# SorF520/D2R

Measured on AMD Instinct MI355X. Metric: samples/sec fwd+bwd, higher is better.
Workload: dtype fp16; 1 GPU; BASELINE configs[1]: synthetic MVSA-Single-style batch, per-GPU batch 32, seq_len 128, 197 image tokens, DR_step 3, 6 cells per routing layer, 3 classes, 12+12 encoder layers, random-init weights, dropout 0; step = fwd+bwd+grad-allreduce+AdamW; global_batch=32, seq_len=128, parallelism=dp1

## Files before the change

d2r_amd/csrc/gemm.hip:

```cpp
#include <stdlib.h>

#include <algorithm>
#include <mutex>
#include <vector>

#include "gemm_args.h"
#include "ktimer.h"

template <typename T, int LAYOUT, int BM, int BN, int WAVES_M, int WAVES_N, int NBUF, bool GROUPED = false>
__global__ __launch_bounds__(256) void gemm_kernel(GemmArgs g, GemmGroup grp) {
  constexpr bool IS_BF16 = sizeof(T) == 2;
  constexpr int BK = IS_BF16 ? 64 : 16;
  constexpr int VEC = 16 / sizeof(T);
  constexpr int NT = 256;
  static_assert(WAVES_M * WAVES_N == 4, "4 waves per workgroup");
  constexpr int WM = BM / WAVES_M, WN = BN / WAVES_N;
  constexpr int TM = WM / 16, TN = WN / 16;
  static_assert(WM % 16 == 0 && WN % 16 == 0, "wave tile must be a multiple of 16");
  constexpr bool A_KCONT = (LAYOUT != D2R_GEMM_TN);
  constexpr bool B_KCONT = (LAYOUT == D2R_GEMM_NT);
  constexpr int LDK = BK + (IS_BF16 ? 8 : 1);
  constexpr int LDA_T = BM + (IS_BF16 ? 8 : 16);
  constexpr int LDB_T = BN + (IS_BF16 ? 8 : 16);
  constexpr int SZ_A = A_KCONT ? BM * LDK : BK * LDA_T;
// ... 292 lines not shown
        if (g.P) store_c(g.P, g.c_dtype, ci, v);
        v = act_apply_cold(g.act, v);
        if (g.R) v += load_c(g.R, g.c_dtype, rz + (int64_t)row * g.ldr + col);
        if (g.beta != 0.f) v += g.beta * load_c(g.C, g.c_dtype, ci);
        store_c(g.C, g.c_dtype, ci, v);
      }
    }
  }
}

__global__ __launch_bounds__(256) void splitk_reduce_kernel(GemmArgs g) {
  const int64_t total = (int64_t)g.M * g.N;
  if (g.dbias) {
    const float* wb = g.ws + (int64_t)g.splits * total;
    for (int64_t m = (int64_t)blockIdx.x * 256 + threadIdx.x; m < g.M; m += (int64_t)gridDim.x * 256) {
      float s = 0.f;
      for (int k = 0; k < g.splits; ++k) s += wb[(int64_t)k * g.M + m];
      g.dbias[m] += s;
    }
  }
  for (int64_t idx = (int64_t)blockIdx.x * 256 + threadIdx.x; idx < total; idx += (int64_t)gridDim.x * 256) {
    float s = 0.f;
    for (int k0 = 0; k0 < g.splits; k0 += 8) {
      float t[8];
#pragma unroll
      for (int u = 0; u < 8; ++u) {
        const int k = k0 + u;
        t[u] = g.ws[(int64_t)(k < g.splits ? k : 0) * total + idx] * (k < g.splits ? 1.f : 0.f);
      }
#pragma unroll
      for (int u = 0; u < 8; ++u) s += t[u];
    }
    const int m = (int)(idx / g.N), n = (int)(idx - (int64_t)m * g.N);
    const int64_t ci = (int64_t)m * g.ldc + n;
    float v = g.alpha * s + (g.bias ? g.bias[n] : 0.f);
    if (g.P) store_c(g.P, g.c_dtype, ci, v);
    v = act_apply_cold(g.act, v);
    if (g.G) v *= act_grad_cold(g.gact, load_c(g.G, g.c_dtype, ci));
    if (g.R) v += load_c(g.R, g.c_dtype, (int64_t)m * g.ldr + n);
    if (g.beta != 0.f) v += g.beta * load_c(g.C, g.c_dtype, ci);
    store_c(g.C, g.c_dtype, ci, v);
  }
}

static int g_nbuf = 1;
static int g_vepi = 1;
static int g_tile = -1;
static int g_xcd = 1;
static int g_wgrad_glds = 1;
static int g_dbg = 0;
static int g_gemm8 = 1;
static int g_group = 1;
static int g_gemm8_wgrad = 1;
static int g_splitk = 1;
static int g_gemm8_min = 150;

thread_local int d2r_gemm_variant_tl = 0;

struct GemmTimerRec {
  int family;
  double flops, bytes;
  hipEvent_t e0, e1;
};
static std::vector<GemmTimerRec> g_timer_recs;
static std::mutex g_timer_mu;
static volatile int g_timer_on = 0;

static thread_local int g_timer_depth = 0;
D2RTimerScope::D2RTimerScope(hipStream_t stream, int fam, double fl, double by) : family(fam), flops(fl), bytes(by), st(stream) {
  if (fam < 10000) d2r_gemm_variant_tl = 0;
  if (g_timer_depth++ > 0) return;
  if (!g_timer_on) return;
  if (hipEventCreate(&e0) != hipSuccess) return;
  if (hipEventCreate(&e1) != hipSuccess) { (void)hipEventDestroy(e0); return; }
  (void)hipEventRecord(e0, st);
  armed = true;
}
D2RTimerScope::~D2RTimerScope() {
  --g_timer_depth;
  if (!armed) return;
  GemmTimerRec rec;
  rec.family = family < 10000 ? family + 100 * d2r_gemm_variant_tl : family;
  rec.flops = flops, rec.bytes = bytes, rec.e0 = e0, rec.e1 = e1;
  (void)hipEventRecord(e1, st);
  std::lock_guard<std::mutex> lk(g_timer_mu);
  g_timer_recs.push_back(rec);
}
typedef D2RTimerScope GemmTimerScope;

extern "C" int d2r_gemm_timer(int on) {
  std::lock_guard<std::mutex> lk(g_timer_mu);
  if (on) {
    for (auto& r : g_timer_recs) (void)hipEventDestroy(r.e0), (void)hipEventDestroy(r.e1);
    g_timer_recs.clear();
  }
  g_timer_on = on ? 1 : 0;
  return D2R_OK;
}

extern "C" int d2r_gemm_timer_read(int* family, double* flops, double* bytes, float* ms, int capacity) {
  std::lock_guard<std::mutex> lk(g_timer_mu);
  int n = 0;
  for (auto& r : g_timer_recs) {
    float t = 0.f;
    if (hipEventSynchronize(r.e1) == hipSuccess && hipEventElapsedTime(&t, r.e0, r.e1) == hipSuccess && n < capacity && family) {
      family[n] = r.family, flops[n] = r.flops, bytes[n] = r.bytes, ms[n] = t;
      ++n;
    }
    (void)hipEventDestroy(r.e0), (void)hipEventDestroy(r.e1);
  }
  const int total = (int)g_timer_recs.size();
  g_timer_recs.clear();
  return family ? n : total;
}
extern "C" void d2r_gemm_tuning(int nbuf, int vepi, int tile) {
  g_nbuf = nbuf & 0xff;
  g_xcd = (nbuf >> 8) & 1 ? 0 : 1;
  g_vepi = vepi;
  if (tile == 100 || tile == 101) g_wgrad_glds = tile - 100;
  else if (tile == 102 || tile == 103) g_gemm8_wgrad = tile - 102;
  else if (tile >= 110 && tile <= 113) g_gemm8 = tile - 110;
  else if (tile == 130 || tile == 131) g_splitk = tile - 130;
  else if (tile == 120 || tile == 121) g_group = tile - 120;
  else if (tile >= 2000) g_dbg = tile - 2000;
  else if (tile >= 1000) g_gemm8_min = tile - 1000;
  else g_tile = tile;
}

template <typename T, int LAYOUT, int BM, int BN, int WM_, int WN_>
static void launch_tile(const GemmArgs& a, int gz, hipStream_t st) {
  dim3 grid(d2r_cdiv(a.N, BN), d2r_cdiv(a.M, BM), gz);
  static const GemmGroup no_group = {};
  if (g_nbuf == 2) hipLaunchKernelGGL((gemm_kernel<T, LAYOUT, BM, BN, WM_, WN_, 2>), grid, dim3(256), 0, st, a, no_group);
  else hipLaunchKernelGGL((gemm_kernel<T, LAYOUT, BM, BN, WM_, WN_, 1>), grid, dim3(256), 0, st, a, no_group);
}

int d2r_gemm_glds_try(const GemmArgs& a, int layout, int batch, int bn, hipStream_t st);
int d2r_gemm8_fwd_ok(const GemmArgs& a, int layout, int batch);
int d2r_gemm8_fwd_launch(const GemmArgs* probs, int n, int layout, hipStream_t st);
int d2r_gemm8_wgrad_ok(int dtype, int M, int N, int K, int64_t lda, int64_t ldb, int64_t ldc, const void* A, const void* B, const void* C);
int d2r_gemm8_wgrad_launch(int dtype, int count, const int* M, const int* N, const int* K, const int64_t* lda, const int64_t* ldb, const int64_t* ldc,
                           const void* const* A, const void* const* B, float* const* C, float* const* dbias, float beta, hipStream_t st);
int d2r_gemm_glds_splitk_plan(const GemmArgs& a, int layout, int batch, size_t ws_bytes, size_t* slab_bytes);
int d2r_gemm_glds_splitk_launch(const GemmArgs& a, int layout, hipStream_t st);
static bool gemm8_pays(const GemmArgs& a) {
  if (g_gemm8 == 2 && (a.act != 0 || a.G != nullptr)) return false;
  if (g_gemm8 == 3 && (a.act != 0 || a.G != nullptr || a.R != nullptr || a.P != nullptr)) return false;
  const int64_t t = (int64_t)d2r_cdiv(a.M, 256) * d2r_cdiv(a.N, 256);
  if (t < g_gemm8_min) return false;
  const int64_t rounds = (t + 255) / 256;
  return t * 100 >= rounds * 256 * 70;
}
static int g_glds = 1;

template <int LAYOUT>
__global__ __launch_bounds__(256) void gemm_skinny_f32_kernel(GemmArgs g) {
  constexpr int MAXS = 12;
  __shared__ float red[4][2][16][17];
  const int tid = threadIdx.x, lane = tid & 63, wave = tid >> 6;
  const int fr = lane & 15, fq = lane >> 4;
  const int z = blockIdx.z, zb = z / g.nh, zh = z - zb * g.nh;
  const float* A = reinterpret_cast<const float*>(g.A) + zb * g.sAb + zh * g.sAh;
  const float* B = reinterpret_cast<const float*>(g.B) + zb * g.sBb + zh * g.sBh;
  const int n0 = blockIdx.x * 16;
  const int col = min(n0 + fr, g.N - 1);
  const int r0 = min(fr, g.M - 1), r1 = min(16 + fr, g.M - 1);
  const bool two = g.M > 16;
  f32x4 acc0 = {0.f, 0.f, 0.f, 0.f}, acc1 = {0.f, 0.f, 0.f, 0.f};
  const int k16 = g.K / 16, per = (k16 + 3) / 4;
  const int kbeg = min(wave * per, k16), kend = min(kbeg + per, k16);
  for (int s0 = kbeg; s0 < kbeg + per; s0 += MAXS) {
    const int ns = max(0, min(MAXS, kend - s0));
    f32x4 a0[MAXS], a1[MAXS], b[MAXS];
#pragma unroll
    for (int s = 0; s < MAXS; ++s) {
      if (s < ns) {
        const int k = (s0 + s) * 16 + fq * 4;
        a0[s] = *reinterpret_cast<const f32x4*>(A + (int64_t)r0 * g.lda + k);
        if (two) a1[s] = *reinterpret_cast<const f32x4*>(A + (int64_t)r1 * g.lda + k);
        if constexpr (LAYOUT == D2R_GEMM_NT) {
          b[s] = *reinterpret_cast<const f32x4*>(B + (int64_t)col * g.ldb + k);
        } else {
#pragma unroll
          for (int j = 0; j < 4; ++j) b[s][j] = B[(int64_t)(k + j) * g.ldb + col];
        }
      }
    }
#pragma unroll
    for (int s = 0; s < MAXS; ++s) {
      if (s < ns) {
#pragma unroll
        for (int j = 0; j < 4; ++j) {
          acc0 = __builtin_amdgcn_mfma_f32_16x16x4f32(a0[s][j], b[s][j], acc0, 0, 0, 0);
          if (two) acc1 = __builtin_amdgcn_mfma_f32_16x16x4f32(a1[s][j], b[s][j], acc1, 0, 0, 0);
        }
// ... 512 lines not shown
  for (int first = 0; first < count; first += D2R_GEMM_GROUP_MAX) {
    const int n = count - first < D2R_GEMM_GROUP_MAX ? count - first : D2R_GEMM_GROUP_MAX;
    GemmGroup grp = {};
    for (int i = 0; i < n; ++i) {
      grp.A[i] = A[first + i], grp.B[i] = B[first + i], grp.C[i] = C[first + i];
      grp.dbias[i] = dbias ? dbias[first + i] : nullptr;
    }
    GemmArgs a = base;
    a.dbias = dbias ? reinterpret_cast<float*>(1) : nullptr;
    if (sizeof(T) == 2 && g_wgrad_glds) {
      GemmArgs b = a;
      b.xcd = g_xcd;
      if (d2r_gemm_glds_wgrad_try(b, grp, n, st)) {
        if (int rc = d2r_check_launch("d2r_gemm_tn_grouped(glds)")) return rc;
        continue;
      }
    }
    dim3 grid(d2r_cdiv(a.N, 64), d2r_cdiv(a.M, 64), n);
    if (a.K >= 1 && a.K <= 64 && (int64_t)a.M * a.N >= 4096) {
      d2r_gemm_variant_tl = 33;
      hipLaunchKernelGGL((gemm_rank_tn_kernel<T, true>), grid, dim3(256), 0, st, a, grp);
      if (int rc = d2r_check_launch("d2r_gemm_tn_grouped(rank-K)")) return rc;
      continue;
    }
    if (grid.x >= 24 && grid.x % 8 == 0) a.xcd = 0;
    d2r_gemm_variant_tl = 21;
    hipLaunchKernelGGL((gemm_kernel<T, D2R_GEMM_TN, 64, 64, 2, 2, 1, true>), grid, dim3(256), 0, st, a, grp);
    if (int rc = d2r_check_launch("d2r_gemm_tn_grouped")) return rc;
  }
  return D2R_OK;
}

static int tn_grouped_same(int dtype, int M, int N, int K, int64_t lda, int64_t ldb, int64_t ldc, const void* const* h_A, const void* const* h_B,
                           float* const* h_C, float* const* h_dbias, int count, float beta, void* stream, bool allow8) {
  D2R_REQUIRE(h_A && h_B && h_C && count >= 0, "d2r_gemm_tn_grouped: null pointer array");
  D2R_REQUIRE(dtype == D2R_F32 || d2r_is16(dtype), "d2r_gemm_tn_grouped: bad dtype %d", dtype);
  D2R_REQUIRE(M >= 1 && N >= 1 && K >= 0 && lda >= M && ldb >= N && ldc >= N, "d2r_gemm_tn_grouped: bad shape");
  if (count == 0) return D2R_OK;
  const int64_t es = (int64_t)d2r_esize(dtype);
  GemmArgs a = {};
  a.M = M, a.N = N, a.K = K, a.nh = 1, a.splits = 1, a.lda = lda, a.ldb = ldb, a.ldc = ldc;
  a.alpha = 1.f, a.beta = beta, a.act = D2R_ACT_NONE, a.c_dtype = D2R_F32, a.dtype = dtype, a.xcd = g_xcd, a.grouped = 1, a.dbg = 0, a.band = 0;
  a.vecA = (lda * es) % 16 == 0, a.vecB = (ldb * es) % 16 == 0, a.vecC = 0;
  for (int i = 0; i < count; ++i) {
    D2R_REQUIRE(h_A[i] && h_B[i] && h_C[i] && (!h_dbias || h_dbias[i]), "d2r_gemm_tn_grouped: null operand in problem %d", i);
    a.vecA &= d2r_aligned16(h_A[i]) ? 1 : 0;
    a.vecB &= d2r_aligned16(h_B[i]) ? 1 : 0;
    for (int j = 0; j < i; ++j) {
      D2R_REQUIRE(h_C[i] != h_C[j], "d2r_gemm_tn_grouped: problems %d and %d write the same C", j, i);
      D2R_REQUIRE(!h_dbias || h_dbias[i] != h_dbias[j], "d2r_gemm_tn_grouped: problems %d and %d write the same dbias", j, i);
    }
  }
  hipStream_t st = reinterpret_cast<hipStream_t>(stream);
  GemmTimerScope timed(st, dtype * 8 + D2R_GEMM_TN * 2 + 1, 2.0 * count * M * N * (double)K,
                       (double)count * (((double)K * M + (double)K * N) * es + 2.0 * M * N * 4.0));
  if (allow8 && g_gemm8_wgrad && d2r_is16(dtype) && (int64_t)count * d2r_cdiv(M, 256) * d2r_cdiv(N, 256) >= 96) {
    bool ok = true;
    for (int i = 0; i < count && ok; ++i) ok = d2r_gemm8_wgrad_ok(dtype, M, N, K, lda, ldb, ldc, h_A[i], h_B[i], h_C[i]) != 0;
    if (ok) {
      std::vector<int> Ms(count, M), Ns(count, N), Ks(count, K);
      std::vector<int64_t> la(count, lda), lb(count, ldb), lc(count, ldc);
      d2r_gemm_variant_tl = 28;
      return d2r_gemm8_wgrad_launch(dtype, count, Ms.data(), Ns.data(), Ks.data(), la.data(), lb.data(), lc.data(), h_A, h_B, h_C, h_dbias, beta, st);
    }
  }
  if (dtype == D2R_BF16) return launch_grouped_tn<bf16_t>(a, h_A, h_B, h_C, h_dbias, count, st);
  if (dtype == D2R_F16) return launch_grouped_tn<f16_t>(a, h_A, h_B, h_C, h_dbias, count, st);
  return launch_grouped_tn<float>(a, h_A, h_B, h_C, h_dbias, count, st);
}

extern "C" int d2r_gemm_tn_grouped(int dtype, int M, int N, int K, int64_t lda, int64_t ldb, int64_t ldc, const void* const* h_A,
                                   const void* const* h_B, float* const* h_C, float* const* h_dbias, int count, float beta, void* stream) {
  return tn_grouped_same(dtype, M, N, K, lda, ldb, ldc, h_A, h_B, h_C, h_dbias, count, beta, stream, true);
}


extern "C" int d2r_gemm_tn_grouped_v(int dtype, int count, const int* M, const int* N, const int* K, const int64_t* lda, const int64_t* ldb,
                                     const int64_t* ldc, const void* const* h_A, const void* const* h_B, float* const* h_C,
                                     float* const* h_dbias, float beta, void* stream) {
  D2R_REQUIRE(count >= 0 && (count == 0 || (M && N && K && lda && ldb && ldc && h_A && h_B && h_C)), "d2r_gemm_tn_grouped_v: null array");
  D2R_REQUIRE(dtype == D2R_F32 || d2r_is16(dtype), "d2r_gemm_tn_grouped_v: bad dtype %d", dtype);
  hipStream_t st = reinterpret_cast<hipStream_t>(stream);
  std::vector<int> wide, rest;
  for (int i = 0; i < count; ++i) {
    D2R_REQUIRE(h_A[i] && h_B[i] && h_C[i] && (!h_dbias || h_dbias[i]), "d2r_gemm_tn_grouped_v: null operand in problem %d", i);
    D2R_REQUIRE(M[i] >= 1 && N[i] >= 1 && K[i] >= 0 && lda[i] >= M[i] && ldb[i] >= N[i] && ldc[i] >= N[i], "d2r_gemm_tn_grouped_v: bad shape in problem %d", i);
    for (int j = 0; j < i; ++j) {
      D2R_REQUIRE(h_C[i] != h_C[j], "d2r_gemm_tn_grouped_v: problems %d and %d write the same C", j, i);
      D2R_REQUIRE(!h_dbias || h_dbias[i] != h_dbias[j], "d2r_gemm_tn_grouped_v: problems %d and %d write the same dbias", j, i);
    }
    const bool w = g_gemm8_wgrad && d2r_gemm8_wgrad_ok(dtype, M[i], N[i], K[i], lda[i], ldb[i], ldc[i], h_A[i], h_B[i], h_C[i]);
    (w ? wide : rest).push_back(i);
  }
  int64_t wtiles = 0;
  for (int i : wide) wtiles += (int64_t)d2r_cdiv(M[i], 256) * d2r_cdiv(N[i], 256);
  if (wtiles < 96) {
    rest.insert(rest.end(), wide.begin(), wide.end());
    wide.clear();
  }
  if (!wide.empty()) {
    const int n = (int)wide.size();
    std::vector<int> Ms(n), Ns(n), Ks(n);
    std::vector<int64_t> la(n), lb(n), lc(n);
    std::vector<const void*> As(n), Bs(n);
    std::vector<float*> Cs(n), Ds(n);
    double flops = 0, bytes = 0;
    for (int k = 0; k < n; ++k) {
      const int i = wide[k];
      Ms[k] = M[i], Ns[k] = N[i], Ks[k] = K[i], la[k] = lda[i], lb[k] = ldb[i], lc[k] = ldc[i], As[k] = h_A[i], Bs[k] = h_B[i], Cs[k] = h_C[i];
      Ds[k] = h_dbias ? h_dbias[i] : nullptr;
      flops += 2.0 * M[i] * N[i] * (double)K[i];
      bytes += ((double)K[i] * M[i] + (double)K[i] * N[i]) * 2.0 + (beta != 0.f ? 2.0 : 1.0) * M[i] * N[i] * 4.0;
    }
    GemmTimerScope timed(st, dtype * 8 + D2R_GEMM_TN * 2 + 1, flops, bytes);
    d2r_gemm_variant_tl = 28;
    if (int rc = d2r_gemm8_wgrad_launch(dtype, n, Ms.data(), Ns.data(), Ks.data(), la.data(), lb.data(), lc.data(), As.data(), Bs.data(), Cs.data(),
                                        h_dbias ? Ds.data() : nullptr, beta, st))
      return rc;
  }
  std::vector<char> done(count, 0);
  for (size_t a = 0; a < rest.size(); ++a) {
    const int i = rest[a];
    if (done[i]) continue;
    std::vector<const void*> As, Bs;
    std::vector<float*> Cs, Ds;
    for (size_t b = a; b < rest.size(); ++b) {
      const int j = rest[b];
      if (done[j] || M[j] != M[i] || N[j] != N[i] || K[j] != K[i] || lda[j] != lda[i] || ldb[j] != ldb[i] || ldc[j] != ldc[i]) continue;
      done[j] = 1;
      As.push_back(h_A[j]), Bs.push_back(h_B[j]), Cs.push_back(h_C[j]), Ds.push_back(h_dbias ? h_dbias[j] : nullptr);
    }
    if (int rc = tn_grouped_same(dtype, M[i], N[i], K[i], lda[i], ldb[i], ldc[i], As.data(), Bs.data(), Cs.data(), h_dbias ? Ds.data() : nullptr,
                                 (int)As.size(), beta, stream, false))
      return rc;
  }
  return D2R_OK;
}


int d2r_gemm_glds_batched_tn_try(const GemmArgs& a, const GemmGroup& grp, int ngroups, hipStream_t st);
int d2r_gemm_tn_batched16(int dtype, int M, int m_store, int N, int K, int64_t lda, int64_t sAb, int64_t ldb, int64_t sBb, int64_t ldc,
                          int64_t sCb, const void* const* A, const void* const* B, void* const* C, int ngroups, int nb, void* stream) {
  D2R_REQUIRE(d2r_is16(dtype) && A && B && C && ngroups >= 1 && ngroups <= D2R_GEMM_GROUP_MAX && nb >= 1, "d2r_gemm_tn_batched16: bad arguments");
  D2R_REQUIRE(m_store >= 1 && m_store <= M && N >= 1 && K >= 1 && lda >= M && ldb >= N && ldc >= N, "d2r_gemm_tn_batched16: bad shape");
  hipStream_t st = reinterpret_cast<hipStream_t>(stream);
  GemmArgs a = {};
  a.M = M, a.m_store = m_store, a.N = N, a.K = K, a.nh = 1, a.splits = 1, a.lda = lda, a.ldb = ldb, a.ldc = ldc, a.sAb = sAb, a.sBb = sBb, a.sCb = sCb;
  a.alpha = 1.f, a.beta = 0.f, a.act = D2R_ACT_NONE, a.c_dtype = dtype, a.dtype = dtype, a.xcd = g_xcd, a.grouped = 1, a.gbatch = nb;
  auto ok16 = [](const void* p, int64_t ld, int64_t sb) { return d2r_aligned16(p) && (ld * 2) % 16 == 0 && (sb * 2) % 16 == 0; };
  a.vecA = a.vecB = a.vecC = 1;
  GemmGroup grp = {};
  for (int i = 0; i < ngroups; ++i) {
    D2R_REQUIRE(A[i] && B[i] && C[i], "d2r_gemm_tn_batched16: null operand in group %d", i);
    a.vecA &= ok16(A[i], lda, sAb) ? 1 : 0, a.vecB &= ok16(B[i], ldb, sBb) ? 1 : 0, a.vecC &= ok16(C[i], ldc, sCb) ? 1 : 0;
    grp.A[i] = A[i], grp.B[i] = B[i], grp.C[i] = C[i];
  }
  {
    GemmTimerScope timed(st, dtype * 8 + D2R_GEMM_TN * 2 + 1, 2.0 * ngroups * nb * (double)m_store * N * K,
                         (double)ngroups * nb * (((double)K * m_store + (double)K * N) * 2.0 + (double)m_store * N * 2.0));
    if (g_glds && d2r_gemm_glds_batched_tn_try(a, grp, ngroups, st)) return d2r_check_launch("d2r_gemm_tn_batched16(glds)");
  }
  for (int i = 0; i < ngroups; ++i) {
    d2r_gemm_desc d = {};
    d.dtype = d.c_dtype = dtype, d.layout = D2R_GEMM_TN, d.act = D2R_ACT_NONE, d.M = m_store, d.N = N, d.K = K, d.nb = nb, d.nh = 1, d.alpha = 1.f;
    d.A = A[i], d.lda = lda, d.sAb = sAb, d.B = B[i], d.ldb = ldb, d.sBb = sBb, d.C = C[i], d.ldc = ldc, d.sCb = sCb;
    if (int rc = d2r_gemm(&d, stream)) return rc;
  }
  return D2R_OK;
}
```

d2r_amd/csrc/gemm8.hip:

```cpp
#include "gemm_args.h"

#ifndef D2R_G8_STAMPS
#define D2R_G8_STAMPS 0
#endif

__device__ __attribute__((aligned(256))) unsigned char d2r_g8_zero_page[256];

namespace {

constexpr int G8_UNIT = 16384;
constexpr int G8_A0 = 0, G8_B0 = G8_UNIT, G8_B1 = 2 * G8_UNIT, G8_A1 = 3 * G8_UNIT, G8_BUF = 4 * G8_UNIT;
constexpr int G8_SMEM = 2 * G8_BUF;

__device__ __forceinline__ int g8_kswz(int k) { return ((k & 3) | ((k >> 1) & 4)) << 1; }

template <int OFF, typename V8>
__device__ __forceinline__ V8 g8_read128(unsigned addr) {
  V8 r;
  asm volatile("ds_read_b128 %0, %1 offset:%2" : "=v"(r) : "v"(addr), "n"(OFF));
  return r;
}
template <int OFF, typename V4>
__device__ __forceinline__ V4 g8_read_tr(unsigned addr) {
  V4 r;
  asm volatile("ds_read_b64_tr_b16 %0, %1 offset:%2" : "=v"(r) : "v"(addr), "n"(OFF));
  return r;
}

__device__ __forceinline__ void g8_barrier() {
  asm volatile("s_barrier" ::: "memory");
  __builtin_amdgcn_sched_barrier(0);
}
__device__ __forceinline__ void g8_lgkm0() {
  asm volatile("s_waitcnt lgkmcnt(0)" ::: "memory");
  __builtin_amdgcn_sched_barrier(0);
}
__device__ __forceinline__ void g8_wait_units(int units) {
  if (units >= 4) asm volatile("s_waitcnt vmcnt(8)" ::: "memory");
  else if (units == 3) asm volatile("s_waitcnt vmcnt(6)" ::: "memory");
  else if (units == 2) asm volatile("s_waitcnt vmcnt(4)" ::: "memory");
  else if (units == 1) asm volatile("s_waitcnt vmcnt(2)" ::: "memory");
  else asm volatile("s_waitcnt vmcnt(0)" ::: "memory");
  __builtin_amdgcn_sched_barrier(0);
}

template <typename E, int LAYOUT, bool BIAS>
__device__ __forceinline__ void g8_main(const E* __restrict__ A, const E* __restrict__ B, int M, int N, int K, int64_t lda, int64_t ldb,
                                        int m0, int n0, unsigned char* smem, f32x4 (&acc)[8][4], f32x4 (&accb)[2], bool do_bias,
                                        unsigned long long* stamps) {
  typedef typename H16<E>::v8 h8;
  typedef typename H16<E>::v4 h4;
  constexpr bool A_KC = LAYOUT != D2R_GEMM_TN, B_KC = LAYOUT == D2R_GEMM_NT;
  constexpr bool RAGGED = LAYOUT == D2R_GEMM_TN;
// ... 172 lines not shown
    G8_MFMA(0, 0, bf0);
    G8_BIAS(0);
    G8_STAMP(sb + 1);
    g8_barrier();
    G8_STAMP(sb + 2);
    G8_READ_B(G8_B1, bf1);
    __builtin_amdgcn_sched_barrier(0);
    if (more1) issueA(1, buf ^ 1, t + 1);
    __builtin_amdgcn_sched_barrier(0);
    g8_wait_units(more1 ? INF : 0);
    g8_barrier();
    G8_STAMP(sb + 3);
    g8_lgkm0();
    G8_MFMA(0, 1, bf1);
    G8_STAMP(sb + 4);
    g8_barrier();
    G8_STAMP(sb + 5);
    G8_READ_A(G8_A1);
    __builtin_amdgcn_sched_barrier(0);
    if (more2) issueA(0, buf, t + 2);
    __builtin_amdgcn_sched_barrier(0);
    g8_barrier();
    G8_STAMP(sb + 6);
    g8_lgkm0();
    G8_MFMA(1, 1, bf1);
    G8_BIAS(1);
    G8_STAMP(sb + 7);
    g8_barrier();
    G8_STAMP(sb + 8);
    if (more2) issueB(0, buf, t + 2);
    __builtin_amdgcn_sched_barrier(0);
    if (more1) g8_wait_units(more2 ? INF : 2);
    g8_barrier();
    G8_STAMP(sb + 9);
    G8_MFMA(1, 0, bf0);
    G8_STAMP(sb + 10);
    g8_barrier();
    G8_STAMP(sb + 11);
  }
  if (wr == 0) g8_barrier();
  G8_STAMP(63);
  if (stamps && blockIdx.x == 0) {
    asm volatile("s_waitcnt vmcnt(0)" ::: "memory");
    stamps[wave * 64 + lane] = ((unsigned long long)st_hi << 32) | st_lo;
  }
#undef G8_STAMP
#undef G8_READ_A
#undef G8_READ_B
#undef G8_MFMA
#undef G8_BIAS
}

constexpr int G8_WMAX = 40;
struct G8ProbW {
  const void* A;
  const void* B;
  float* C;
  float* dbias;
  int M, N, K, lda, ldb, ldc, tn, pad;
};
struct G8GroupW {
  int nprob, ntiles;
  float beta;
  int xcd;
  unsigned long long* stamps;
  int tile_end[G8_WMAX];
  G8ProbW p[G8_WMAX];
};

__device__ __forceinline__ int g8_xcd_remap(int id, int nwg, int enable) {
  if (!enable || nwg < 16) return id;
  const int q = nwg >> 3, r = nwg & 7, xcd = id & 7, k = id >> 3;
  return (xcd < r ? xcd * (q + 1) : r * (q + 1) + (xcd - r) * q) + k;
}

template <typename E>
__global__ __launch_bounds__(512) void gemm8_wgrad_kernel(const G8GroupW g) {
  __shared__ __attribute__((aligned(1024))) unsigned char smem[G8_SMEM];
  const int L = g8_xcd_remap(blockIdx.x, g.ntiles, g.xcd);
  int lo = 0, hi = g.nprob - 1;
  while (lo < hi) {
    const int mid = (lo + hi) >> 1;
    if (L < g.tile_end[mid]) hi = mid;
    else lo = mid + 1;
  }
  const int z = __builtin_amdgcn_readfirstlane(lo);
  const G8ProbW& P = g.p[z];
  const int first = z ? g.tile_end[z - 1] : 0;
  const int rem = L - first, tile_m = rem / P.tn, tile_n = rem - tile_m * P.tn;
  const int m0 = tile_m * 256, n0 = tile_n * 256;
  const int M = P.M, N = P.N;
  f32x4 acc[8][4], accb[2];
#pragma unroll
  for (int i = 0; i < 8; ++i)
#pragma unroll
    for (int j = 0; j < 4; ++j) acc[i][j] = f32x4{0.f, 0.f, 0.f, 0.f};
  accb[0] = accb[1] = f32x4{0.f, 0.f, 0.f, 0.f};
  const bool do_bias = P.dbias != nullptr && tile_n == 0;
  g8_main<E, D2R_GEMM_TN, true>(reinterpret_cast<const E*>(P.A), reinterpret_cast<const E*>(P.B), M, N, P.K, P.lda, P.ldb, m0, n0, smem, acc, accb,
                                     do_bias, D2R_G8_STAMPS ? g.stamps : nullptr);

  const int lane = threadIdx.x & 63, wave = __builtin_amdgcn_readfirstlane(threadIdx.x >> 6), wr = wave >> 2, wc = wave & 3;
  const int fr = lane & 15, fq = lane >> 4;
  float* C = P.C;
  const int64_t ldc = P.ldc;
  const float beta = g.beta;
#pragma unroll
  for (int mh = 0; mh < 2; ++mh) {
    f32x4 old[4][4];
    if (beta != 0.f) {
#pragma unroll
      for (int i = 0; i < 4; ++i) {
        const int row = min(m0 + wr * 128 + mh * 64 + i * 16 + fr, M - 1);
#pragma unroll
        for (int nj = 0; nj < 4; ++nj) {
          const int col = min(n0 + wc * 64 + (nj >> 1) * 32 + (nj & 1) * 16 + fq * 4, N - 4);
          old[i][nj] = *reinterpret_cast<const f32x4*>(C + (int64_t)row * ldc + col);
        }
      }
    }
#pragma unroll
    for (int i = 0; i < 4; ++i) {
      const int row = m0 + wr * 128 + mh * 64 + i * 16 + fr;
#pragma unroll
      for (int nj = 0; nj < 4; ++nj) {
        const int col = n0 + wc * 64 + (nj >> 1) * 32 + (nj & 1) * 16 + fq * 4;
        f32x4 v = acc[mh * 4 + i][nj];
        if (beta != 0.f) v = f32x4{v[0] + beta * old[i][nj][0], v[1] + beta * old[i][nj][1], v[2] + beta * old[i][nj][2], v[3] + beta * old[i][nj][3]};
        if (row < M && col + 4 <= N) *reinterpret_cast<f32x4*>(C + (int64_t)row * ldc + col) = v;
      }
    }
  }
// ... 121 lines not shown
void launch_fwd(const G8GroupF& g, int layout, hipStream_t st) {
  if (layout == D2R_GEMM_NT) hipLaunchKernelGGL((gemm8_fwd_kernel<E, D2R_GEMM_NT>), dim3(g.ntiles), dim3(512), 0, st, g);
  else hipLaunchKernelGGL((gemm8_fwd_kernel<E, D2R_GEMM_NN>), dim3(g.ntiles), dim3(512), 0, st, g);
}

}

static unsigned long long* g8_stamps = nullptr;
extern "C" void d2r_gemm8_debug_stamps(unsigned long long* dst) { g8_stamps = dst; }
int d2r_gemm8_fwd_ok(const GemmArgs& a, int layout, int batch) {
  if (!d2r_is16(a.dtype) || a.c_dtype != a.dtype || batch != 1 || layout == D2R_GEMM_TN) return 0;
  if (a.K % 64 != 0 || a.K < 128 || a.M < 256 || a.N < 256 || a.N % 8 != 0) return 0;
  if (!a.vecA || !a.vecB || !a.vecC || a.dbias) return 0;
  return 1;
}

static void g8_fill_prob(G8ProbF& p, const GemmArgs& a) {
  p.A = a.A, p.B = a.B, p.C = a.C, p.bias = a.bias, p.R = a.R, p.P = a.P, p.G = a.G;
  p.M = a.M, p.N = a.N, p.K = a.K, p.lda = (int)a.lda, p.ldb = (int)a.ldb, p.ldc = (int)a.ldc, p.ldr = (int)a.ldr;
  p.tn = d2r_cdiv(a.N, 256);
  p.alpha = a.alpha, p.beta = a.beta, p.act = a.act, p.gact = a.gact, p.pad = 0;
  const int64_t panel = (int64_t)256 * a.K * 2;
  int band = (int)((int64_t)(1536 << 10) / (panel > 0 ? panel : 1));
  if (band < 2) band = 2;
  p.band = (p.tn > band && (int64_t)p.tn * panel > (3 << 20)) ? band : 0;
}

int d2r_gemm8_fwd_launch(const GemmArgs* probs, int n, int layout, hipStream_t st) {
  if (n < 1 || n > G8_FMAX) return d2r_fail(D2R_ERR_INVALID, "d2r_gemm8_fwd_launch: %d problems (1..%d)", n, G8_FMAX);
  G8GroupF g = {};
  g.nprob = n, g.xcd = 1;
  int tiles = 0;
  for (int i = 0; i < n; ++i) {
    g8_fill_prob(g.p[i], probs[i]);
    tiles += d2r_cdiv(probs[i].M, 256) * g.p[i].tn;
    g.tile_end[i] = tiles;
  }
  for (int i = n; i < G8_FMAX; ++i) g.tile_end[i] = tiles;
  g.ntiles = tiles;
  g.stamps = g8_stamps;
  if (probs[0].dtype == D2R_F16) launch_fwd<f16_t>(g, layout, st);
  else launch_fwd<bf16_t>(g, layout, st);
  return d2r_check_launch("d2r_gemm8(fwd)");
}

int d2r_gemm8_wgrad_ok(int dtype, int M, int N, int K, int64_t lda, int64_t ldb, int64_t ldc, const void* A, const void* B, const void* C) {
  if (!d2r_is16(dtype) || M < 128 || N < 128 || K < 128 || M % 8 != 0 || N % 8 != 0) return 0;
  if ((lda * 2) % 16 != 0 || (ldb * 2) % 16 != 0 || (ldc * 4) % 16 != 0) return 0;
  if (!d2r_aligned16(A) || !d2r_aligned16(B) || !d2r_aligned16(C)) return 0;
  if (lda >= ((int64_t)1 << 31) || ldb >= ((int64_t)1 << 31) || ldc >= ((int64_t)1 << 31)) return 0;
  return 1;
}

int d2r_gemm8_wgrad_launch(int dtype, int count, const int* M, const int* N, const int* K, const int64_t* lda, const int64_t* ldb, const int64_t* ldc,
                           const void* const* A, const void* const* B, float* const* C, float* const* dbias, float beta, hipStream_t st) {
  for (int first = 0; first < count; first += G8_WMAX) {
    const int n = count - first < G8_WMAX ? count - first : G8_WMAX;
    G8GroupW g = {};
    g.nprob = n, g.beta = beta, g.xcd = 1;
    int tiles = 0;
    for (int i = 0; i < n; ++i) {
      const int s = first + i;
      G8ProbW& p = g.p[i];
      p.A = A[s], p.B = B[s], p.C = C[s], p.dbias = dbias ? dbias[s] : nullptr;
      p.M = M[s], p.N = N[s], p.K = K[s], p.lda = (int)lda[s], p.ldb = (int)ldb[s], p.ldc = (int)ldc[s];
      p.tn = d2r_cdiv(N[s], 256), p.pad = 0;
      tiles += d2r_cdiv(M[s], 256) * p.tn;
      g.tile_end[i] = tiles;
    }
    for (int i = n; i < G8_WMAX; ++i) g.tile_end[i] = tiles;
    g.ntiles = tiles;
    g.stamps = g8_stamps;
    if (dtype == D2R_F16) hipLaunchKernelGGL((gemm8_wgrad_kernel<f16_t>), dim3(tiles), dim3(512), 0, st, g);
    else hipLaunchKernelGGL((gemm8_wgrad_kernel<bf16_t>), dim3(tiles), dim3(512), 0, st, g);
    if (int rc = d2r_check_launch("d2r_gemm8(wgrad)")) return rc;
  }
  return D2R_OK;
}

extern "C" int d2r_gemm8_probe_fwd(int dtype, int layout, int M, int N, int K, const void* A, int64_t lda, const void* B, int64_t ldb, void* C,
                                   int64_t ldc, const float* bias, int act, int nrep, void* stream) {
  GemmArgs a = {};
  a.A = A, a.B = B, a.C = C, a.bias = bias, a.M = M, a.N = N, a.K = K, a.lda = lda, a.ldb = ldb, a.ldc = ldc, a.ldr = ldc;
  a.alpha = 1.f, a.beta = 0.f, a.act = act, a.dtype = dtype, a.c_dtype = dtype, a.vecA = a.vecB = a.vecC = 1;
  if (!d2r_gemm8_fwd_ok(a, layout, 1)) return d2r_fail(D2R_ERR_INVALID, "d2r_gemm8_probe_fwd: shape not eligible");
  GemmArgs probs[G8_FMAX];
  if (nrep < 1 || nrep > G8_FMAX) return d2r_fail(D2R_ERR_INVALID, "d2r_gemm8_probe_fwd: nrep");
  for (int i = 0; i < nrep; ++i) probs[i] = a;
  return d2r_gemm8_fwd_launch(probs, nrep, layout, reinterpret_cast<hipStream_t>(stream));
}
```

d2r_amd/csrc/gemm_args.h:

```cpp
#pragma once
#include "common.h"

typedef __attribute__((ext_vector_type(8))) __bf16 bf16x8;
typedef __attribute__((ext_vector_type(4))) __bf16 bf16x4;
typedef __attribute__((ext_vector_type(8))) _Float16 f16x8;
typedef __attribute__((ext_vector_type(4))) _Float16 f16x4;
typedef __attribute__((ext_vector_type(4))) float f32x4;

template <typename T> struct H16;
template <> struct H16<bf16_t> {
  typedef bf16x8 v8;
  typedef bf16x4 v4;
  static constexpr int DT = D2R_BF16;
  static __device__ __forceinline__ f32x4 mfma32(v8 a, v8 b, f32x4 c) { return __builtin_amdgcn_mfma_f32_16x16x32_bf16(a, b, c, 0, 0, 0); }
  static __device__ __forceinline__ f32x4 mfma16(v4 a, v4 b, f32x4 c) { return __builtin_amdgcn_mfma_f32_16x16x16bf16_1k(a, b, c, 0, 0, 0); }
  static __device__ __forceinline__ v4 tr_read(const bf16_t* lds) {
    typedef __attribute__((address_space(3))) v4 lds_v4;
    return __builtin_amdgcn_ds_read_tr16_b64_v4bf16((lds_v4*)lds);
  }
};
template <> struct H16<f16_t> {
  typedef f16x8 v8;
  typedef f16x4 v4;
  static constexpr int DT = D2R_F16;
  static __device__ __forceinline__ f32x4 mfma32(v8 a, v8 b, f32x4 c) { return __builtin_amdgcn_mfma_f32_16x16x32_f16(a, b, c, 0, 0, 0); }
  static __device__ __forceinline__ f32x4 mfma16(v4 a, v4 b, f32x4 c) { return __builtin_amdgcn_mfma_f32_16x16x16f16(a, b, c, 0, 0, 0); }
  static __device__ __forceinline__ v4 tr_read(const f16_t* lds) {
    typedef __attribute__((ext_vector_type(4))) short i16x4;
    typedef __attribute__((address_space(3))) i16x4 lds_v4;
    return __builtin_bit_cast(v4, __builtin_amdgcn_ds_read_tr16_b64_v4i16((lds_v4*)lds));
  }
};
template <> struct H16<float> {
  typedef bf16x8 v8;
  typedef bf16x4 v4;
  static constexpr int DT = D2R_F32;
};
template <typename T> struct Out16 { typedef T type; };
template <> struct Out16<float> { typedef bf16_t type; };

extern thread_local int d2r_gemm_variant_tl;

constexpr int D2R_GEMM_GROUP_MAX = 32;
struct GemmGroup {
  const void* A[D2R_GEMM_GROUP_MAX];
  const void* B[D2R_GEMM_GROUP_MAX];
  void* C[D2R_GEMM_GROUP_MAX];
  float* dbias[D2R_GEMM_GROUP_MAX];
};

struct GemmArgs {
  const void* A;
  const void* B;
  void* C;
  const float* bias;
  const void* R;
  void* P;
  float* ws;
  float* dbias;
  const void* G;
  int gact;
  int grouped;
  int M, N, K, nh, splits, tiles_per_split;
  int64_t lda, ldb, ldc, ldr;
  int64_t sAb, sAh, sBb, sBh, sCb, sCh, sRb, sRh, sBiasB;
  float alpha, beta;
  int act, c_dtype, vecA, vecB, vecC, xcd;
  int dtype;
  int band;
  int gbatch;
  int m_store;
  int dbg;
  unsigned long long* ts;
  unsigned* kflags;
};

template <typename T, int VEC>
__device__ __forceinline__ Pack<T, VEC> load_guard(const T* rowp, int c0, int climit, bool row_ok, bool vec_ok) {
  Pack<T, VEC> r;
  if (row_ok && vec_ok && c0 + VEC <= climit) {
    r = ld_pack<T, VEC>(rowp + c0);
  } else {
#pragma unroll
    for (int j = 0; j < VEC; ++j) r.v[j] = (row_ok && c0 + j < climit) ? rowp[c0 + j] : from_f<T>(0.f);
  }
  return r;
}

__device__ __forceinline__ void xcd_tile(int enable, int& tile_m, int& tile_n, int band = 0) {
  const int gx = gridDim.x, gy = gridDim.y, nwg = gx * gy;
  int id = blockIdx.y * gx + blockIdx.x;
  if (enable && gridDim.z == 1 && nwg >= 16) {
    const int q = nwg >> 3, r = nwg & 7, xcd = id & 7, k = id >> 3;
    id = (xcd < r ? xcd * (q + 1) : r * (q + 1) + (xcd - r) * q) + k;
  }
  if (band > 0 && band < gx) {
    const int per_band = gy * band;
    const int b = id / per_band;
    const int first = b * band;
    const int w = min(band, gx - first);
    const int rem = id - b * per_band;
// ... 265 lines not shown
```

d2r_amd/csrc/gemm_glds.hip:

```cpp
#include "gemm_args.h"

#ifndef D2R_GEMM_PROBES
#define D2R_GEMM_PROBES 0
#endif


template <int CH>
__device__ __forceinline__ int kswz(int k) {
  if constexpr (CH >= 16) return ((k & 3) | ((k >> 1) & 4)) << 1;
  else return (((k >> 1) & 1) | ((k >> 2) & 2)) << 1;
}

template <int CH>
__device__ __forceinline__ int kpos(int c, int k) { return c ^ kswz<CH>(k); }

template <typename E, int LAYOUT, int BN, int NWN, int PIPE, int MODE, int NWM, bool SPLITK = false>
__device__ __forceinline__ void gemm_glds_body(GemmArgs g, const GemmGroup& grp, int tile_m, int tile_n, int z, int split = 0) {
  constexpr bool WGRAD = MODE == 1;
  constexpr bool RAGGED = MODE != 0;
  typedef typename H16<E>::v8 h8;
  typedef typename H16<E>::v4 h4;
  constexpr int BM = 64 * NWM, BK = 64, NW = NWM * NWN;
  constexpr bool A_KCONT = (LAYOUT != D2R_GEMM_TN);
  constexpr bool B_KCONT = (LAYOUT == D2R_GEMM_NT);
// ... 643 lines not shown
  }
  if (bn == 128) {
    dim3 grid(d2r_cdiv(a.N, 128), d2r_cdiv(a.M, 128));
    if (pipe) hipLaunchKernelGGL((gemm_glds_kernel<E, LAYOUT, 128, 2, 1>), grid, dim3(256), 0, st, a, no_group);
    else hipLaunchKernelGGL((gemm_glds_kernel<E, LAYOUT, 128>), grid, dim3(256), 0, st, a, no_group);
  } else {
    dim3 grid(d2r_cdiv(a.N, 64), d2r_cdiv(a.M, 128));
    if (pipe) hipLaunchKernelGGL((gemm_glds_kernel<E, LAYOUT, 64, 2, 1>), grid, dim3(256), 0, st, a, no_group);
    else hipLaunchKernelGGL((gemm_glds_kernel<E, LAYOUT, 64>), grid, dim3(256), 0, st, a, no_group);
  }
}

static unsigned long long* g_gemm_stamps = nullptr;
extern "C" void d2r_gemm_debug_stamps(unsigned long long* dst) { g_gemm_stamps = dst; }

int d2r_gemm_glds_try(const GemmArgs& a, int layout, int batch, int bn, hipStream_t st) {
  if (!d2r_is16(a.dtype) || batch != 1 || a.K % 64 != 0 || a.K < 128 || a.M < 128 || a.N < 64) return 0;
  if ((bn % 1000) == 129 && a.N < 128) return 0;
  if (!a.vecA || !a.vecB) return 0;
  if (a.G && !(a.vecC && a.c_dtype == a.dtype)) return 0;
  const bool a_strided = layout == D2R_GEMM_TN, b_strided = layout != D2R_GEMM_NT;
  if ((a_strided && a.M % 8 != 0) || (b_strided && a.N % 8 != 0)) return 0;
  const bool f16 = a.dtype == D2R_F16;
  GemmArgs ab = a;
  ab.ts = g_gemm_stamps;
  {
    const int bnw = (bn % 1000) == 64 ? 64 : 128;
    const int gx = d2r_cdiv(a.N, bnw);
    const int64_t panel = (int64_t)bnw * a.K * 2;
    int band = (int)((int64_t)(1536 << 10) / (panel > 0 ? panel : 1));
    if (band < 2) band = 2;
    ab.band = (a.K <= 1536 && gx > band && gx * panel > (3 << 20)) ? band : 0;
  }
  d2r_gemm_variant_tl = ((bn % 1000) == 64 ? 1 : (bn % 1000) == 128 ? 2 : 3) + (bn >= 1000 ? 10 : 0);
  switch (layout) {
    case D2R_GEMM_NT: f16 ? launch_glds<f16_t, D2R_GEMM_NT>(ab, bn, st) : launch_glds<bf16_t, D2R_GEMM_NT>(ab, bn, st); break;
    case D2R_GEMM_NN: f16 ? launch_glds<f16_t, D2R_GEMM_NN>(ab, bn, st) : launch_glds<bf16_t, D2R_GEMM_NN>(ab, bn, st); break;
    case D2R_GEMM_TN: f16 ? launch_glds<f16_t, D2R_GEMM_TN>(ab, bn, st) : launch_glds<bf16_t, D2R_GEMM_TN>(ab, bn, st); break;
    default: return 0;
  }
  return 1;
}


int d2r_gemm_glds_wgrad_try(const GemmArgs& a, const GemmGroup& grp, int n, hipStream_t st) {
  if (!d2r_is16(a.dtype) || a.K < 128 || a.M < 128 || a.N < 128 || !a.vecA || !a.vecB || a.M % 8 != 0 || a.N % 8 != 0) return 0;
  d2r_gemm_variant_tl = 20;
  dim3 grid(d2r_cdiv(a.N, 128), d2r_cdiv(a.M, 128), n);
  if (a.dtype == D2R_F16) hipLaunchKernelGGL((gemm_glds_kernel<f16_t, D2R_GEMM_TN, 128, 2, 1, 1>), grid, dim3(256), 0, st, a, grp);
  else hipLaunchKernelGGL((gemm_glds_kernel<bf16_t, D2R_GEMM_TN, 128, 2, 1, 1>), grid, dim3(256), 0, st, a, grp);
  return 1;
}


int d2r_gemm_glds_batched_tn_try(const GemmArgs& a, const GemmGroup& grp, int ngroups, hipStream_t st) {
  if (!d2r_is16(a.dtype) || a.c_dtype != a.dtype || !a.vecA || !a.vecB || !a.vecC || a.M % 8 != 0 || a.N % 8 != 0 || a.M < 8 || a.N < 8 || a.K < 1) return 0;
  if (ngroups < 1 || ngroups > D2R_GEMM_GROUP_MAX || a.gbatch < 1 || (int64_t)ngroups * a.gbatch > 65535) return 0;
  dim3 grid(d2r_cdiv(a.N, 128), d2r_cdiv(a.M, 128), ngroups * a.gbatch);
  d2r_gemm_variant_tl = 22;
  if (a.dtype == D2R_F16) hipLaunchKernelGGL((gemm_glds_kernel<f16_t, D2R_GEMM_TN, 128, 2, 1, 2>), grid, dim3(256), 0, st, a, grp);
  else hipLaunchKernelGGL((gemm_glds_kernel<bf16_t, D2R_GEMM_TN, 128, 2, 1, 2>), grid, dim3(256), 0, st, a, grp);
  return 1;
}
```

Measured before the change: 1605 samples/s.

## Carve wgrad tail-wave tiles into a finer 128-tile kernel and sort by K

In the grouped wgrad path, the 256x256 gemm8 kernel no longer launches every tile. When the tile count leaves a small partial last wave relative to the CU count, the leftover tiles are moved to a separate glds kernel that splits each 256 tile into four 128x128 blocks, aiming to shrink the tail-wave imbalance. Problems are also stable-sorted by K depth, and the XCD remap becomes segment-aware so that tiles with equal K are spread evenly across XCDs. This adds a second launch and more host-side setup per call, and the tail kernel may be slower per flop.

```diff
diff --git a/d2r_amd/csrc/gemm.hip b/d2r_amd/csrc/gemm.hip
--- a/d2r_amd/csrc/gemm.hip
+++ b/d2r_amd/csrc/gemm.hip
@@ -368,6 +368,7 @@
 static int g_gemm8 = 1;
 static int g_group = 1;
 static int g_gemm8_wgrad = 1;
+static int g_wgrad_tail = 1;
 static int g_splitk = 1;
 static int g_gemm8_min = 150;
 
@@ -435,6 +436,7 @@
   g_vepi = vepi;
   if (tile == 100 || tile == 101) g_wgrad_glds = tile - 100;
   else if (tile == 102 || tile == 103) g_gemm8_wgrad = tile - 102;
+  else if (tile == 104 || tile == 105) g_wgrad_tail = tile - 104;
   else if (tile >= 110 && tile <= 113) g_gemm8 = tile - 110;
   else if (tile == 130 || tile == 131) g_splitk = tile - 130;
   else if (tile == 120 || tile == 121) g_group = tile - 120;
@@ -456,7 +458,8 @@
 int d2r_gemm8_fwd_launch(const GemmArgs* probs, int n, int layout, hipStream_t st);
 int d2r_gemm8_wgrad_ok(int dtype, int M, int N, int K, int64_t lda, int64_t ldb, int64_t ldc, const void* A, const void* B, const void* C);
 int d2r_gemm8_wgrad_launch(int dtype, int count, const int* M, const int* N, const int* K, const int64_t* lda, const int64_t* ldb, const int64_t* ldc,
-                           const void* const* A, const void* const* B, float* const* C, float* const* dbias, float beta, hipStream_t st);
+                           const void* const* A, const void* const* B, float* const* C, float* const* dbias, float beta, int tail, int family,
+                           hipStream_t st);
 int d2r_gemm_glds_splitk_plan(const GemmArgs& a, int layout, int batch, size_t ws_bytes, size_t* slab_bytes);
 int d2r_gemm_glds_splitk_launch(const GemmArgs& a, int layout, hipStream_t st);
 static bool gemm8_pays(const GemmArgs& a) {
@@ -1075,18 +1078,18 @@
     }
   }
   hipStream_t st = reinterpret_cast<hipStream_t>(stream);
-  GemmTimerScope timed(st, dtype * 8 + D2R_GEMM_TN * 2 + 1, 2.0 * count * M * N * (double)K,
-                       (double)count * (((double)K * M + (double)K * N) * es + 2.0 * M * N * 4.0));
   if (allow8 && g_gemm8_wgrad && d2r_is16(dtype) && (int64_t)count * d2r_cdiv(M, 256) * d2r_cdiv(N, 256) >= 96) {
     bool ok = true;
     for (int i = 0; i < count && ok; ++i) ok = d2r_gemm8_wgrad_ok(dtype, M, N, K, lda, ldb, ldc, h_A[i], h_B[i], h_C[i]) != 0;
     if (ok) {
       std::vector<int> Ms(count, M), Ns(count, N), Ks(count, K);
       std::vector<int64_t> la(count, lda), lb(count, ldb), lc(count, ldc);
-      d2r_gemm_variant_tl = 28;
-      return d2r_gemm8_wgrad_launch(dtype, count, Ms.data(), Ns.data(), Ks.data(), la.data(), lb.data(), lc.data(), h_A, h_B, h_C, h_dbias, beta, st);
-    }
-  }
+      return d2r_gemm8_wgrad_launch(dtype, count, Ms.data(), Ns.data(), Ks.data(), la.data(), lb.data(), lc.data(), h_A, h_B, h_C, h_dbias, beta,
+                                    g_wgrad_tail, dtype * 8 + D2R_GEMM_TN * 2 + 1, st);
+    }
+  }
+  GemmTimerScope timed(st, dtype * 8 + D2R_GEMM_TN * 2 + 1, 2.0 * count * M * N * (double)K,
+                       (double)count * (((double)K * M + (double)K * N) * es + 2.0 * M * N * 4.0));
   if (dtype == D2R_BF16) return launch_grouped_tn<bf16_t>(a, h_A, h_B, h_C, h_dbias, count, st);
   if (dtype == D2R_F16) return launch_grouped_tn<f16_t>(a, h_A, h_B, h_C, h_dbias, count, st);
   return launch_grouped_tn<float>(a, h_A, h_B, h_C, h_dbias, count, st);
@@ -1127,18 +1130,13 @@
     std::vector<int64_t> la(n), lb(n), lc(n);
     std::vector<const void*> As(n), Bs(n);
     std::vector<float*> Cs(n), Ds(n);
-    double flops = 0, bytes = 0;
     for (int k = 0; k < n; ++k) {
       const int i = wide[k];
       Ms[k] = M[i], Ns[k] = N[i], Ks[k] = K[i], la[k] = lda[i], lb[k] = ldb[i], lc[k] = ldc[i], As[k] = h_A[i], Bs[k] = h_B[i], Cs[k] = h_C[i];
       Ds[k] = h_dbias ? h_dbias[i] : nullptr;
-      flops += 2.0 * M[i] * N[i] * (double)K[i];
-      bytes += ((double)K[i] * M[i] + (double)K[i] * N[i]) * 2.0 + (beta != 0.f ? 2.0 : 1.0) * M[i] * N[i] * 4.0;
-    }
-    GemmTimerScope timed(st, dtype * 8 + D2R_GEMM_TN * 2 + 1, flops, bytes);
-    d2r_gemm_variant_tl = 28;
+    }
     if (int rc = d2r_gemm8_wgrad_launch(dtype, n, Ms.data(), Ns.data(), Ks.data(), la.data(), lb.data(), lc.data(), As.data(), Bs.data(), Cs.data(),
-                                        h_dbias ? Ds.data() : nullptr, beta, st))
+                                        h_dbias ? Ds.data() : nullptr, beta, g_wgrad_tail, dtype * 8 + D2R_GEMM_TN * 2 + 1, st))
       return rc;
   }
   std::vector<char> done(count, 0);
diff --git a/d2r_amd/csrc/gemm8.hip b/d2r_amd/csrc/gemm8.hip
--- a/d2r_amd/csrc/gemm8.hip
+++ b/d2r_amd/csrc/gemm8.hip
@@ -1,4 +1,7 @@
+#include <algorithm>
+
 #include "gemm_args.h"
+#include "ktimer.h"
 
 #ifndef D2R_G8_STAMPS
 #define D2R_G8_STAMPS 0
@@ -277,6 +280,7 @@
 }
 
 constexpr int G8_WMAX = 40;
+constexpr int G8_SEGS = 4;
 struct G8ProbW {
   const void* A;
   const void* B;
@@ -289,6 +293,7 @@
   float beta;
   int xcd;
   unsigned long long* stamps;
+  int nseg, seg_end[G8_SEGS];
   int tile_end[G8_WMAX];
   G8ProbW p[G8_WMAX];
 };
@@ -299,10 +304,26 @@
   return (xcd < r ? xcd * (q + 1) : r * (q + 1) + (xcd - r) * q) + k;
 }
 
+__device__ __forceinline__ int g8_seg_remap(int id, const G8GroupW& g) {
+  if (!g.xcd || g.ntiles < 16) return id;
+  const int x = id & 7, k = id >> 3;
+  auto cnt = [](int e, int y) { return (e - y + 7) >> 3; };
+  int s = 0, start = 0, before = 0;
+  while (s + 1 < g.nseg && k >= cnt(g.seg_end[s], x)) {
+    start = g.seg_end[s];
+    before = cnt(start, x);
+    ++s;
+  }
+  const int end = g.seg_end[s];
+  int off = 0;
+  for (int y = 0; y < x; ++y) off += cnt(end, y) - cnt(start, y);
+  return start + off + (k - before);
+}
+
 template <typename E>
 __global__ __launch_bounds__(512) void gemm8_wgrad_kernel(const G8GroupW g) {
   __shared__ __attribute__((aligned(1024))) unsigned char smem[G8_SMEM];
-  const int L = g8_xcd_remap(blockIdx.x, g.ntiles, g.xcd);
+  const int L = g8_seg_remap(blockIdx.x, g);
   int lo = 0, hi = g.nprob - 1;
   while (lo < hi) {
     const int mid = (lo + hi) >> 1;
@@ -530,27 +551,103 @@
   return 1;
 }
 
+int d2r_gemm_glds_wgrad_tail_launch(int dtype, const GemmWgradTailGroup& tg, hipStream_t st);
+
+static int g8_cu_count() {
+  static int cus[64] = {};
+  int dev = 0;
+  if (hipGetDevice(&dev) != hipSuccess || dev < 0 || dev >= 64) return 0;
+  if (cus[dev] == 0) {
+    int v = 0;
+    if (hipDeviceGetAttribute(&v, hipDeviceAttributeMultiprocessorCount, dev) != hipSuccess || v < 1) return 0;
+    cus[dev] = v;
+  }
+  return cus[dev];
+}
+
+constexpr int G8_TAIL_NUM = 1, G8_TAIL_DEN = 2;
 int d2r_gemm8_wgrad_launch(int dtype, int count, const int* M, const int* N, const int* K, const int64_t* lda, const int64_t* ldb, const int64_t* ldc,
-                           const void* const* A, const void* const* B, float* const* C, float* const* dbias, float beta, hipStream_t st) {
+                           const void* const* A, const void* const* B, float* const* C, float* const* dbias, float beta, int tail, int family,
+                           hipStream_t st) {
+  const int cus = tail ? g8_cu_count() : 0;
   for (int first = 0; first < count; first += G8_WMAX) {
     const int n = count - first < G8_WMAX ? count - first : G8_WMAX;
-    G8GroupW g = {};
-    g.nprob = n, g.beta = beta, g.xcd = 1;
-    int tiles = 0;
+    int order[G8_WMAX], ntile[G8_WMAX], tiles = 0;
+    for (int i = 0; i < n; ++i) {
+      order[i] = first + i;
+      ntile[i] = d2r_cdiv(M[first + i], 256) * d2r_cdiv(N[first + i], 256);
+      tiles += ntile[i];
+    }
+    if (tail) std::stable_sort(order, order + n, [&](int a, int b) { return d2r_cdiv(K[a], 64) > d2r_cdiv(K[b], 64); });
+    int carve = 0;
+    if (tail && cus > 0 && tiles / cus >= 2) {
+      const int rem = tiles % cus;
+      if (rem > 0 && rem * G8_TAIL_DEN <= cus * G8_TAIL_NUM) carve = rem;
+    }
+    GemmWgradTailGroup tg = {};
+    double flops_all = 0, bytes_all = 0, flops_tail = 0;
     for (int i = 0; i < n; ++i) {
       const int s = first + i;
-      G8ProbW& p = g.p[i];
+      flops_all += 2.0 * M[s] * N[s] * (double)K[s];
+      bytes_all += ((double)K[s] * M[s] + (double)K[s] * N[s]) * 2.0 + (beta != 0.f ? 2.0 : 1.0) * M[s] * N[s] * 4.0;
+    }
+    int wide_tiles[G8_WMAX];
+    for (int i = 0; i < n; ++i) wide_tiles[i] = ntile[order[i] - first];
+    {
+      int left = carve;
+      for (int i = n - 1; i >= 0 && left > 0; --i) {
+        if (tg.nprob == D2R_WGRAD_TAIL_MAX) break;
+        const int s = order[i], take = left < wide_tiles[i] ? left : wide_tiles[i];
+        GemmWgradTailProb& p = tg.p[tg.nprob];
+        p.A = A[s], p.B = B[s], p.C = C[s], p.dbias = dbias ? dbias[s] : nullptr;
+        p.M = M[s], p.N = N[s], p.K = K[s], p.lda = (int)lda[s], p.ldb = (int)ldb[s], p.ldc = (int)ldc[s];
+        p.tn = d2r_cdiv(N[s], 256), p.t0 = wide_tiles[i] - take;
+        for (int t = p.t0; t < wide_tiles[i]; ++t) {
+          const int tm = t / p.tn, tc = t - tm * p.tn;
+          const int mh = M[s] - tm * 256 < 256 ? M[s] - tm * 256 : 256, nw = N[s] - tc * 256 < 256 ? N[s] - tc * 256 : 256;
+          flops_tail += 2.0 * mh * nw * (double)K[s];
+        }
+        tg.ntiles += take;
+        tg.tile_end[tg.nprob++] = tg.ntiles;
+        wide_tiles[i] -= take;
+        left -= take;
+      }
+      if (left > 0) {
+        tg = GemmWgradTailGroup{};
+        flops_tail = 0;
+        for (int i = 0; i < n; ++i) wide_tiles[i] = ntile[order[i] - first];
+      }
+    }
+    if (tg.ntiles > 0) {
+      for (int i = tg.nprob; i < D2R_WGRAD_TAIL_MAX; ++i) tg.tile_end[i] = tg.ntiles;
+      tg.beta = beta;
+      D2RTimerScope timed(st, family, flops_tail, bytes_all * (flops_tail / flops_all));
+      if (int rc = d2r_gemm_glds_wgrad_tail_launch(dtype, tg, st)) return rc;
+    }
+    G8GroupW g = {};
+    g.beta = beta, g.xcd = 1;
+    int wt = 0, prev_nk = -1;
+    for (int i = 0; i < n; ++i) {
+      if (wide_tiles[i] == 0) continue;
+      const int s = order[i];
+      G8ProbW& p = g.p[g.nprob];
       p.A = A[s], p.B = B[s], p.C = C[s], p.dbias = dbias ? dbias[s] : nullptr;
       p.M = M[s], p.N = N[s], p.K = K[s], p.lda = (int)lda[s], p.ldb = (int)ldb[s], p.ldc = (int)ldc[s];
       p.tn = d2r_cdiv(N[s], 256), p.pad = 0;
-      tiles += d2r_cdiv(M[s], 256) * p.tn;
-      g.tile_end[i] = tiles;
-    }
-    for (int i = n; i < G8_WMAX; ++i) g.tile_end[i] = tiles;
-    g.ntiles = tiles;
+      const int nk = d2r_cdiv(K[s], 64);
+      if (tail && prev_nk >= 0 && nk != prev_nk && g.nseg < G8_SEGS - 1) g.seg_end[g.nseg++] = wt;
+      prev_nk = nk;
+      wt += wide_tiles[i];
+      g.tile_end[g.nprob++] = wt;
+    }
+    for (int i = g.nprob; i < G8_WMAX; ++i) g.tile_end[i] = wt;
+    g.seg_end[g.nseg++] = wt;
+    g.ntiles = wt;
     g.stamps = g8_stamps;
-    if (dtype == D2R_F16) hipLaunchKernelGGL((gemm8_wgrad_kernel<f16_t>), dim3(tiles), dim3(512), 0, st, g);
-    else hipLaunchKernelGGL((gemm8_wgrad_kernel<bf16_t>), dim3(tiles), dim3(512), 0, st, g);
+    D2RTimerScope timed(st, family, flops_all - flops_tail, bytes_all * (1.0 - flops_tail / flops_all));
+    d2r_gemm_variant_tl = 28;
+    if (dtype == D2R_F16) hipLaunchKernelGGL((gemm8_wgrad_kernel<f16_t>), dim3(wt), dim3(512), 0, st, g);
+    else hipLaunchKernelGGL((gemm8_wgrad_kernel<bf16_t>), dim3(wt), dim3(512), 0, st, g);
     if (int rc = d2r_check_launch("d2r_gemm8(wgrad)")) return rc;
   }
   return D2R_OK;
diff --git a/d2r_amd/csrc/gemm_args.h b/d2r_amd/csrc/gemm_args.h
--- a/d2r_amd/csrc/gemm_args.h
+++ b/d2r_amd/csrc/gemm_args.h
@@ -47,6 +47,22 @@
   const void* B[D2R_GEMM_GROUP_MAX];
   void* C[D2R_GEMM_GROUP_MAX];
   float* dbias[D2R_GEMM_GROUP_MAX];
+};
+
+constexpr int D2R_WGRAD_TAIL_MAX = 16;
+struct GemmWgradTailProb {
+  const void* A;
+  const void* B;
+  float* C;
+  float* dbias;
+  int M, N, K, lda, ldb, ldc, tn, t0;
+};
+struct GemmWgradTailGroup {
+  int nprob, ntiles;
+  float beta;
+  int pad;
+  int tile_end[D2R_WGRAD_TAIL_MAX];
+  GemmWgradTailProb p[D2R_WGRAD_TAIL_MAX];
 };
 
 struct GemmArgs {
diff --git a/d2r_amd/csrc/gemm_glds.hip b/d2r_amd/csrc/gemm_glds.hip
--- a/d2r_amd/csrc/gemm_glds.hip
+++ b/d2r_amd/csrc/gemm_glds.hip
@@ -719,6 +719,39 @@
   return 1;
 }
 
+template <typename E>
+__global__ __launch_bounds__(256) void gemm_glds_wgrad_tail_kernel(GemmArgs g, GemmWgradTailGroup tg) {
+  const int L = blockIdx.x >> 2, sub = blockIdx.x & 3;
+  int lo = 0, hi = tg.nprob - 1;
+  while (lo < hi) {
+    const int mid = (lo + hi) >> 1;
+    if (L < tg.tile_end[mid]) hi = mid;
+    else lo = mid + 1;
+  }
+  const int e = __builtin_amdgcn_readfirstlane(lo);
+  const GemmWgradTailProb& P = tg.p[e];
+  const int w = P.t0 + L - (e ? tg.tile_end[e - 1] : 0);
+  const int wm = w / P.tn, wn = w - wm * P.tn;
+  const int tile_m = wm * 2 + (sub >> 1), tile_n = wn * 2 + (sub & 1);
+  if (tile_m * 128 >= P.M || tile_n * 128 >= P.N) return;
+  g.M = P.M, g.N = P.N, g.K = P.K, g.lda = P.lda, g.ldb = P.ldb, g.ldc = P.ldc, g.beta = tg.beta;
+  GemmGroup grp;
+  grp.A[0] = P.A, grp.B[0] = P.B, grp.C[0] = P.C, grp.dbias[0] = P.dbias;
+  gemm_glds_body<E, D2R_GEMM_TN, 128, 2, 1, 1, 2>(g, grp, tile_m, tile_n, 0);
+}
+
+int d2r_gemm_glds_wgrad_tail_launch(int dtype, const GemmWgradTailGroup& tg, hipStream_t st) {
+  if (tg.nprob < 1 || tg.nprob > D2R_WGRAD_TAIL_MAX || tg.ntiles < 1)
+    return d2r_fail(D2R_ERR_INVALID, "d2r_gemm_glds_wgrad_tail_launch: %d entries, %d tiles", tg.nprob, tg.ntiles);
+  GemmArgs a = {};
+  a.nh = 1, a.splits = 1, a.alpha = 1.f, a.act = D2R_ACT_NONE, a.c_dtype = D2R_F32, a.dtype = dtype, a.grouped = 1, a.vecA = a.vecB = 1;
+  a.dbias = reinterpret_cast<float*>(1);
+  d2r_gemm_variant_tl = 20;
+  if (dtype == D2R_F16) hipLaunchKernelGGL((gemm_glds_wgrad_tail_kernel<f16_t>), dim3(tg.ntiles * 4), dim3(256), 0, st, a, tg);
+  else hipLaunchKernelGGL((gemm_glds_wgrad_tail_kernel<bf16_t>), dim3(tg.ntiles * 4), dim3(256), 0, st, a, tg);
+  return d2r_check_launch("d2r_gemm8(wgrad tail)");
+}
+
 
 int d2r_gemm_glds_batched_tn_try(const GemmArgs& a, const GemmGroup& grp, int ngroups, hipStream_t st) {
   if (!d2r_is16(a.dtype) || a.c_dtype != a.dtype || !a.vecA || !a.vecB || !a.vecC || a.M % 8 != 0 || a.N % 8 != 0 || a.M < 8 || a.N < 8 || a.K < 1) return 0;
```

Result: no change. 1601 samples/s, median of 2 (-0.2%).
